# alessiodevoto/peekvit

Measured on AMD Instinct MI355X. Metric: images/sec ViT-B/16 fwd @ batch 2048, 224x224, higher is better.
Workload: dtype f16; 1 GPU; vit_b_16 forward, batch 2048/GPU, 224x224; global_batch=2048, parallelism=replicas x1 (batch-sharded, no collective), precision_mode=auto, streams=1, operands=IEEE fp16 operands, fp32 accumulate (same MFMA rate as bf16), range-guarded, range_guard_fallbacks=0

## Files before the change

peekvit_amd/csrc/pv_gemm.hip:

```cpp
#include "pv_rows.h"
#include "../../include/peekvit_hip_moe.h"
#include "pv_gelu_table.h"
#include <type_traits>
#include <cstdlib>

typedef __attribute__((ext_vector_type(8))) short s16x8;

#ifndef PV_STORE_NT
#define PV_STORE_NT 3
#endif
#define PV_STORE16(ptr, val) do { if (PV_STORE_NT & 1) __builtin_nontemporal_store((val), (ptr)); else *(ptr) = (val); } while (0)
#define PV_STORE32(ptr, val) do { if (PV_STORE_NT & 2) __builtin_nontemporal_store((val), (ptr)); else *(ptr) = (val); } while (0)
#ifndef PV_PF_MODE
#define PV_PF_MODE 2
#endif
#ifndef PV_EPI_PIPE
#define PV_EPI_PIPE 1
#endif

__device__ __forceinline__ float pv_fma_s(float a, float b, float c) {
    float r;
    asm("v_fma_f32 %0, %1, %2, %3" : "=v"(r) : "v"(a), "v"(b), "v"(c));
    return r;
}
// ... 113 lines not shown
    int fr_big;
    int gm;
    int gc;
    uint32_t* range_flag;
    float* rowsq_out;
    int res_scaled;
    int k_last;
    float* colsum_partial;
    uint16_t* x16_out;
    float* rowstat_out;
    const float* fold_stat;
    const float* fold_c1;
    const float* fold_c2;
    int ksplit;
    int k_slice;
    int64_t split_stride;
    const float* ln_gamma;
    const float* ln_beta;
    const float* ln_row_scale;
    uint16_t* ln_out;
    float ln_eps;
    const int* row_map;
    int map_rows;
#ifdef PV_STAMPS
    unsigned long long* dbg;
#endif
};

#ifdef PV_STAMPS
static unsigned long long* g_pv_dbg = nullptr;
extern "C" void pv_debug_set_stamp_buffer(void* p) { g_pv_dbg = (unsigned long long*)p; }
#define PV_STAMP(i)                                                                                  \
    do {                                                                                             \
        __builtin_amdgcn_sched_barrier(0);                                                           \
        unsigned long long t_;                                                                       \
        asm volatile("s_memtime %0\n\ts_waitcnt lgkmcnt(0)" : "=s"(t_)::"memory");                    \
        __builtin_amdgcn_sched_barrier(0);                                                           \
        if (threadIdx.x == 0 && p.dbg) p.dbg[pv_stamp_slot * 16 + (i)] = t_;                         \
    } while (0)
#else
#define PV_STAMP(i)
#endif

template <int AUX = 0>
__device__ __forceinline__ void pv_glds16(const void* gsrc, void* lds_wave_base) {
    __builtin_amdgcn_global_load_lds((const __attribute__((address_space(1))) void*)gsrc,
// ... 338 lines not shown
    static PvPerDevice attr_set;
    const int lds = 2 * 2 * G1_TILE_BYTES;
    if (attr_set.first_use()) (void)hipFuncSetAttribute(reinterpret_cast<const void*>(pv_patch_embed_kernel), hipFuncAttributeMaxDynamicSharedMemorySize, lds);
    PV_LAUNCH(pv_patch_embed_kernel, dim3((unsigned)(p.tiles_m * p.tiles_n)), dim3(256), lds, (hipStream_t)stream, p, gm);
    return pv_check_launch();
}

template <int EPI>
static int pv_launch_gemm128(const GemmDev& p, hipStream_t stream) {
    static PvPerDevice attr_set;
    const int lds = 2 * 2 * G1_TILE_BYTES;
    if (attr_set.first_use()) {
        (void)hipFuncSetAttribute(reinterpret_cast<const void*>(pv_gemm128_kernel<EPI>), hipFuncAttributeMaxDynamicSharedMemorySize, lds);
    }
    PV_LAUNCH(pv_gemm128_kernel<EPI>, dim3((unsigned)(p.tiles_m * p.tiles_n * (p.ksplit > 1 ? p.ksplit : 1))), dim3(256), lds, stream, p);
    return pv_check_launch();
}

constexpr int G2_BM = 256, G2_BN = 256, G2_BK = 64;
constexpr int G2_HALF = 128 * G2_BK * 2;
constexpr int G2_BUF = 4 * G2_HALF;
constexpr int G2_LDS = 2 * G2_BUF;

template <int EPI, bool PF = false, bool FULL = false, bool PERM = false>
__device__ __forceinline__ void pv_gemm256_tile(const GemmDev& p, char* smem, const int m0, const int n0, const bool first = true,
                                                const bool has_next = false, const int nm0 = 0, const int nn0 = 0, const int wid_pf = 0, const int slot_pf = 0) {
    int tid_ = threadIdx.x;
    if (PF) {
        int l_;
        asm volatile("v_mbcnt_lo_u32_b32 %0, -1, 0\n\tv_mbcnt_hi_u32_b32 %0, -1, %0" : "=v"(l_));
        tid_ = wid_pf * 64 + l_;
    }
    int tid = tid_, lane = tid & 63;
    const int wid = PF ? wid_pf : __builtin_amdgcn_readfirstlane(tid >> 6);
    const int wr = wid >> 2, wc = wid & 3;
#ifdef PV_STAMPS
    const size_t pv_stamp_slot = PF ? (size_t)slot_pf : (size_t)blockIdx.x;
#endif
    constexpr int PFM = PV_PF_MODE;
    constexpr int PF_BIAS_BASE = G2_LDS + ((EPI == PV_EPI_BIAS_GELU_BF16 || EPI == PV_EPI_BIAS_GELU_SPLIT_BF16 || EPI == PV_EPI_BIAS_GELU_PAIR_BF16) ? PV_GELU_CUB_N * PV_GELU_CUB_REP * 16 : 0) + 4096;
    PV_STAMP(14);
#ifdef PV_STAMPS
    if (threadIdx.x == 0 && p.dbg) { unsigned long long rt_; asm volatile("s_memrealtime %0\n\ts_waitcnt lgkmcnt(0)" : "=s"(rt_)::"memory"); p.dbg[pv_stamp_slot * 16 + 13] = rt_; }
#endif

    const int srow = wid * 8 + (lane >> 3);
    const int schunk = (lane & 7) ^ ((lane >> 3) & 7);
    const char* const a_blk = reinterpret_cast<const char*>(p.A + (int64_t)m0 * p.lda);
    const char* const w_blk = reinterpret_cast<const char*>(p.W + (int64_t)n0 * p.ldw);
// ... 12 lines not shown
    char* const lds_piece = smem + wid * 1024;
    auto stage_a = [&](int buf, int h, int kt) {
        const char* src = a_blk + kt * (G2_BK * 2);
        pv_glds16<PV_GEMM_A_AUX>(src + oa[h][0], lds_piece + buf * G2_BUF + h * G2_HALF);
        pv_glds16<PV_GEMM_A_AUX>(src + oa[h][1], lds_piece + buf * G2_BUF + h * G2_HALF + 8192);
    };
    auto stage_b = [&](int buf, int h, int kt) {
        const char* src = w_blk + kt * (G2_BK * 2);
        pv_glds16<PV_GEMM_W_AUX>(src + ow[h][0], lds_piece + buf * G2_BUF + (2 + h) * G2_HALF);
        pv_glds16<PV_GEMM_W_AUX>(src + ow[h][1], lds_piece + buf * G2_BUF + (2 + h) * G2_HALF + 8192);
    };
    auto stage_next_piece = [&](int tm0, int tn0, int pc) __attribute__((always_inline)) {
        if (pc == 8) {
            if (p.bias && wid < 4) {
                const int c_ = tn0 + wid * 64 + lane < p.N ? tn0 + wid * 64 + lane : p.N - 1;
                __builtin_amdgcn_global_load_lds((const __attribute__((address_space(1))) void*)(p.bias + c_),
                                                 (__attribute__((address_space(3))) void*)(smem + PF_BIAS_BASE + wid * 256), 4, 0, 0);
            }
            return;
        }
        const int h = (pc >> 1) & 1, jj = pc & 1;
        const int sr = wid * 8 + (lane >> 3), sc = (lane & 7) ^ ((lane >> 3) & 7);
        if (pc < 4) {
            const char* const na = reinterpret_cast<const char*>(p.A + (int64_t)tm0 * p.lda);
            int ra = h * 128 + jj * 64 + sr; ra = tm0 + ra < p.M ? ra : p.M - 1 - tm0;
            pv_glds16<PV_GEMM_A_AUX>(na + (uint32_t)(ra * (int)p.lda + sc * 8) * 2u, lds_piece + h * G2_HALF + jj * 8192);
        } else {
            const char* const nw = reinterpret_cast<const char*>(p.W + (int64_t)tn0 * p.ldw);
            const int q = jj * 64 + sr;
            int rw = h * 128 + (q & ~31) + (((q & 15) >> 2) << 3) + (((q >> 4) & 1) << 2) + (q & 3);
            rw = tn0 + rw < p.N ? rw : p.N - 1 - tn0;
            pv_glds16<PV_GEMM_W_AUX>(nw + (uint32_t)(rw * (int)p.ldw + sc * 8) * 2u, lds_piece + (2 + h) * G2_HALF + jj * 8192);
        }
    };

    typedef __attribute__((address_space(3))) const char lds_cc;
    const int frow = (lane & 15) * 128;
    const int fx0 = ((lane >> 4) ^ (lane & 7)) << 4;
    lds_cc* const lds0 = (lds_cc*)smem;
    lds_cc* a_rd[2][2];
    lds_cc* b_rd[2][2];
#pragma unroll
    for (int b = 0; b < 2; ++b)
#pragma unroll
        for (int ks = 0; ks < 2; ++ks) {
            a_rd[b][ks] = lds0 + b * G2_BUF + wr * G2_HALF + frow + (fx0 ^ (ks << 6));
            b_rd[b][ks] = lds0 + b * G2_BUF + (2 + (wc >> 1)) * G2_HALF + (wc & 1) * 8192 + frow + (fx0 ^ (ks << 6));
            asm volatile("" : "+v"(a_rd[b][ks]));
            asm volatile("" : "+v"(b_rd[b][ks]));
        }

    int en0 = n0 + wc * 64 + ((lane >> 4) << 3);
    f32x4 acc[4][8];
    if (!PF) {
#pragma unroll
        for (int i = 0; i < 4; ++i) {
            f32x4 b4 = {0.f, 0.f, 0.f, 0.f};
            if (p.bias && en0 + (i >> 1) * 32 + (i & 1) * 4 < p.N) b4 = *reinterpret_cast<const f32x4*>(p.bias + en0 + (i >> 1) * 32 + (i & 1) * 4);
#pragma unroll
            for (int j = 0; j < 8; ++j) acc[i][j] = b4;
        }
    }
    bf16x8 af[2][4][2];
    bf16x8 bfr[2][2];

#define G2_READ_A(BUF, MH)                                                                                  \
    _Pragma("unroll") for (int t_ = 0; t_ < 4; ++t_) _Pragma("unroll") for (int ks_ = 0; ks_ < 2; ++ks_)  \
        af[MH][t_][ks_] = *reinterpret_cast<const __attribute__((address_space(3))) bf16x8*>(a_rd[BUF][ks_] + ((MH) * 4 + t_) * 2048);
#define G2_READ_B(BUF, NH)                                                                                  \
    _Pragma("unroll") for (int t_ = 0; t_ < 2; ++t_) _Pragma("unroll") for (int ks_ = 0; ks_ < 2; ++ks_)  \
        bfr[t_][ks_] = *reinterpret_cast<const __attribute__((address_space(3))) bf16x8*>(b_rd[BUF][ks_] + ((NH) * 2 + t_) * 2048);
#define G2_SYNC_LOADS()                                  \
    asm volatile("s_waitcnt lgkmcnt(0)" ::: "memory");   \
    __builtin_amdgcn_s_barrier();                        \
    __builtin_amdgcn_sched_barrier(0);
#define G2_MFMA(MH, NH)                                                                                              \
    __builtin_amdgcn_s_setprio(1);                                                                                   \
    _Pragma("unroll") for (int ks_ = 0; ks_ < 2; ++ks_) _Pragma("unroll") for (int n_ = 0; n_ < 2; ++n_)            \
        _Pragma("unroll") for (int m_ = 0; m_ < 4; ++m_)                                                            \
            acc[(NH) * 2 + n_][(MH) * 4 + m_] = PV_MFMA_16x16x32(                            \
                bfr[n_][ks_], af[MH][m_][ks_], acc[(NH) * 2 + n_][(MH) * 4 + m_], 0, 0, 0);                     \
    __builtin_amdgcn_s_setprio(0);                                                                                   \
    __builtin_amdgcn_sched_barrier(0);                                                                               \
    __builtin_amdgcn_s_barrier();                                                                                    \
    __builtin_amdgcn_sched_barrier(0);

    auto ktile = [&](auto buf_c, auto sb_c, auto sa_c, int kt) {
        constexpr int BUF = decltype(buf_c)::value;
        constexpr bool SB = decltype(sb_c)::value, SA = decltype(sa_c)::value;
        G2_READ_B(BUF, 0)
        __builtin_amdgcn_sched_barrier(0);
        G2_READ_A(BUF, 0)
        if (SB) stage_b(BUF ^ 1, 0, kt + 1);
        G2_SYNC_LOADS()
        G2_MFMA(0, 0)
        G2_READ_A(BUF, 1)
        if (SB) stage_b(BUF ^ 1, 1, kt + 1);
        G2_SYNC_LOADS()
        G2_MFMA(1, 0)
        G2_READ_B(BUF, 1)
        if (SA) stage_a(BUF, 0, kt + 2);
        G2_SYNC_LOADS()
        G2_MFMA(1, 1)
        if (SA) {
            stage_a(BUF, 1, kt + 2);
            asm volatile("s_waitcnt vmcnt(4)" ::: "memory");
        } else {
            asm volatile("s_waitcnt vmcnt(0)" ::: "memory");
        }
        G2_SYNC_LOADS()
        G2_MFMA(0, 1)
    };
    using B0 = std::integral_constant<int, 0>;
    using B1 = std::integral_constant<int, 1>;
    using T = std::true_type;
    using F = std::false_type;

    const int nk = p.K / G2_BK;
    if (PF) __builtin_assume(nk >= 4);
    PV_STAMP(0);
#ifdef PV_STAMPS
    if (threadIdx.x == 0 && p.dbg) { unsigned long long rt_; asm volatile("s_memrealtime %0\n\ts_waitcnt lgkmcnt(0)" : "=s"(rt_)::"memory"); p.dbg[pv_stamp_slot * 16 + 6] = rt_; }
#endif
    const bool own_tile0 = !PF || !PFM || first;
    if (PF && (first || !PFM) && p.bias && wid < 4) {
        const int c_ = n0 + wid * 64 + lane < p.N ? n0 + wid * 64 + lane : p.N - 1;
        __builtin_amdgcn_global_load_lds((const __attribute__((address_space(1))) void*)(p.bias + c_),
                                         (__attribute__((address_space(3))) void*)(smem + PF_BIAS_BASE + wid * 256), 4, 0, 0);
    }
    if (own_tile0) { stage_a(0, 0, 0); stage_a(0, 1, 0); stage_b(0, 0, 0); stage_b(0, 1, 0); }
    stage_a(1, 0, 1); stage_a(1, 1, 1);
    constexpr bool HAS_TAB = EPI == PV_EPI_BIAS_GELU_BF16 || EPI == PV_EPI_BIAS_GELU_SPLIT_BF16 || EPI == PV_EPI_BIAS_GELU_PAIR_BF16;
    constexpr int NTAB = HAS_TAB ? 2 : 0;
    if (HAS_TAB && own_tile0) {
#pragma unroll
        for (int i = 0; i < NTAB; ++i)
            pv_glds16(reinterpret_cast<const char*>(pv_gelu_cub) + (i * 512 + tid) * 16,
                      smem + G2_LDS + (i * 512 + wid * 64) * 16);
    }
    const bool fold_dma = PV_EPI_PIPE && (EPI == PV_EPI_BIAS_BF16 || EPI == PV_EPI_BIAS_GELU_BF16) && p.fold_stat != nullptr;
    if (fold_dma) {
        constexpr int FOLD_BASE = G2_LDS + (EPI == PV_EPI_BIAS_GELU_BF16 ? PV_GELU_CUB_N * PV_GELU_CUB_REP * 16 : 0);
        const int r_ = m0 + (tid >> 1) < p.M ? m0 + (tid >> 1) : p.M - 1;
        __builtin_amdgcn_global_load_lds((const __attribute__((address_space(1))) void*)(p.fold_stat + 2 * (int64_t)r_ + (tid & 1)),
                                         (__attribute__((address_space(3))) void*)(smem + FOLD_BASE + wid * 256), 4, 0, 0);
        const int c_ = n0 + (tid & 255) < p.N ? n0 + (tid & 255) : p.N - 1;
        __builtin_amdgcn_global_load_lds((const __attribute__((address_space(1))) void*)((tid < 256 ? p.fold_c1 : p.fold_c2) + c_),
                                         (__attribute__((address_space(3))) void*)(smem + FOLD_BASE + 2048 + wid * 256), 4, 0, 0);
    }
    if (own_tile0) {
        const int inflight = 4 + NTAB + (fold_dma ? 2 : 0);
        if (inflight == 4) asm volatile("s_waitcnt vmcnt(4)" ::: "memory");
        else if (inflight == 6) asm volatile("s_waitcnt vmcnt(6)" ::: "memory");
        else if (inflight == 8) asm volatile("s_waitcnt vmcnt(8)" ::: "memory");
        else asm volatile("s_waitcnt vmcnt(10)" ::: "memory");
        __builtin_amdgcn_s_barrier();
    }
    __builtin_amdgcn_sched_barrier(0);
    PV_STAMP(1);
    if (PF) {
#pragma unroll
        for (int i = 0; i < 4; ++i) {
            f32x4 b4 = {0.f, 0.f, 0.f, 0.f};
            if (p.bias) b4 = *reinterpret_cast<const __attribute__((address_space(3))) f32x4*>((const __attribute__((address_space(3))) char*)smem + PF_BIAS_BASE + (wc * 64 + ((lane >> 4) << 3) + (i >> 1) * 32 + (i & 1) * 4) * 4);
#pragma unroll
            for (int j = 0; j < 8; ++j) acc[i][j] = b4;
        }
    }
    if (wr == 1) __builtin_amdgcn_s_barrier();

    int kt = 0;
    for (; kt + 4 <= nk; kt += 2) {
        ktile(B0{}, T{}, T{}, kt);
        ktile(B1{}, T{}, T{}, kt + 1);
    }
    ktile(B0{}, T{}, F{}, kt);
    ktile(B1{}, F{}, F{}, kt + 1);
    if (wr == 0) __builtin_amdgcn_s_barrier();
    PV_STAMP(2);
#undef G2_READ_A
#undef G2_READ_B
#undef G2_SYNC_LOADS
#undef G2_MFMA

    typedef __attribute__((address_space(3))) char lds_c;
    lds_c* const cimg = (lds_c*)smem;
    if (PF) {
        asm volatile("v_mbcnt_lo_u32_b32 %0, -1, 0\n\tv_mbcnt_hi_u32_b32 %0, -1, %0" : "=v"(lane));
        tid = wid * 64 + lane;
        en0 = n0 + wc * 64 + ((lane >> 4) << 3);
    }
    const int g = lane >> 4, i16 = lane & 15;
    const bool pf_next = PF && PFM && has_next;
    if (PFM == 1 && pf_next) {
#pragma unroll
        for (int pc = 0; pc < 9; ++pc) stage_next_piece(nm0, nn0, pc);
    }
    if (PV_EPI_PIPE && (EPI == PV_EPI_BIAS_BF16 || EPI == PV_EPI_BIAS_GELU_BF16 || EPI == PV_EPI_BIAS_GELU_PAIR_BF16)) {
        float vmax = 0.f;
        const bool fold = p.fold_stat != nullptr;
        constexpr int FOLD_BASE = G2_LDS + (EPI != PV_EPI_BIAS_BF16 ? PV_GELU_CUB_N * PV_GELU_CUB_REP * 16 : 0);
        constexpr bool PAIR2 = EPI == PV_EPI_BIAS_GELU_PAIR_BF16;
        constexpr int NU = PAIR2 ? 32 : 16;
        if (fold) {
            f32x4 k1[2][2], k2[2][2];
#pragma unroll
            for (int u = 0; u < 2; ++u)
#pragma unroll
                for (int hh = 0; hh < 2; ++hh) {
                    const int col = wc * 64 + u * 32 + g * 8 + hh * 4;
                    k1[u][hh] = *reinterpret_cast<const __attribute__((address_space(3))) f32x4*>(cimg + FOLD_BASE + 2048 + col * 4);
                    k2[u][hh] = *reinterpret_cast<const __attribute__((address_space(3))) f32x4*>(cimg + FOLD_BASE + 3072 + col * 4);
                }
#pragma unroll
            for (int mt = 0; mt < 8; ++mt) {
                const pv_f32x2_t st = *reinterpret_cast<const __attribute__((address_space(3))) pv_f32x2_t*>(cimg + FOLD_BASE + (wr * 128 + mt * 16 + i16) * 8);
                const float f_mean = st[0], f_rstd = st[1];
#pragma unroll
                for (int u = 0; u < 2; ++u)
#pragma unroll
                    for (int e = 0; e < 4; ++e) {
                        acc[2 * u][mt][e] = fmaf(f_rstd, fmaf(-f_mean, k1[u][0][e], acc[2 * u][mt][e]), k2[u][0][e]);
                        acc[2 * u + 1][mt][e] = fmaf(f_rstd, fmaf(-f_mean, k1[u][1][e], acc[2 * u + 1][mt][e]), k2[u][1][e]);
                    }
            }
        }
        PV_STAMP(8);
        const uint32_t tabc = (uint32_t)(uintptr_t)((const __attribute__((address_space(3))) f32x4*)(cimg + G2_LDS) + i16) - 0x40000000u;
        const bool ocol_ok = n0 + (lane & 31) * 8 < p.N;
        const int rb_row0 = (EPI == PV_EPI_BIAS_GELU_PAIR_BF16 ? ((wid >> 1) & 1) * 128 + (wid & 1) * 8 : (wid >> 2) * 128 + (wid & 3) * 8) + (lane >> 5);
        lds_c* const img = cimg + G2_BUF;
        const int rb_lrow0 = (wid >> 2) * 32 + (wid & 3) * 8 + (lane >> 5);
        uint32_t rb_addr[4];
#pragma unroll
        for (int j = 0; j < 4; ++j) {
            const int row = rb_lrow0 + 2 * j;
            rb_addr[j] = (uint32_t)(uintptr_t)img + row * 512 + (((lane & 31) ^ (row & 7)) << 4);
        }
        f32x4 cf[2][8];
        u32x4 rb[4];
        auto acc_unit = [&](int vn) -> int { return PAIR2 ? vn >> 1 : vn; };
        auto cf_slot = [&](int vn) -> int { return acc_unit(vn) & 1; };
        auto unit_x = [&](int vn, int e) -> float { const int n = acc_unit(vn); return acc[2 * (n & 1) + (e >> 2)][n >> 1][e & 3]; };
        auto is_gelu = [&](int vn) -> bool { return EPI == PV_EPI_BIAS_GELU_BF16 || PAIR2; };
        auto gathers = [&](int vn) -> bool { return EPI == PV_EPI_BIAS_GELU_BF16 || (PAIR2 && (vn & 1) == 0); };
        auto is_deriv = [&](int vn) -> bool { return PAIR2 && (vn & 1) == 1; };
        auto issue = [&](int vn) __attribute__((always_inline)) {
            if (gathers(vn)) {
#pragma unroll
                for (int e = 0; e < 8; e += 2) {
                    uint32_t b0, b1;
                    pv_gelu_bits2(unit_x(vn, e), unit_x(vn, e + 1), b0, b1);
                    asm volatile("ds_read_b128 %0, %1" : "=v"(cf[cf_slot(vn)][e]) : "v"((b0 << 8) + tabc));
// ... 81 lines not shown
                wait_unit(vn, PAIR2 ? vn + 2 < NU : (vn + 1 < NU && gathers(vn + 1)), vq > 0 && (vn & 3) == 0);
                finish(vn);
                if (PFM == 1 && vn == 4 && pf_next) asm volatile("s_waitcnt vmcnt(0)" ::: "memory");
                if (vq > 0) store_row(vq - 1, vn & 3);
                if ((vn & 3) == 3) {
                    asm volatile("s_waitcnt lgkmcnt(0)" ::: "memory");
                    if (vq < 4) { PV_STAMP(9 + vq); }
                    __builtin_amdgcn_s_barrier();
                    __builtin_amdgcn_sched_barrier(0);
#pragma unroll
                    for (int j = 0; j < 4; ++j)
                        asm volatile("ds_read_b128 %0, %1 offset:%2" : "=v"(rb[j]) : "v"(rb_addr[j]), "n"((vq & 1) * 32768));
                }
            }
            asm volatile("s_waitcnt lgkmcnt(0)" : "+v"(rb[0]), "+v"(rb[1]), "+v"(rb[2]), "+v"(rb[3]));
#pragma unroll
            for (int j = 0; j < 4; ++j) store_row(NU / 4 - 1, j);
        }
        pv_range_commit(vmax, p.range_flag);
    } else
    if (EPI == PV_EPI_BIAS_BF16 || EPI == PV_EPI_BIAS_GELU_BF16 || EPI == PV_EPI_BIAS_GELU_SPLIT_BF16 || EPI == PV_EPI_BIAS_GELU_PAIR_BF16) {
        constexpr bool SPLIT = EPI == PV_EPI_BIAS_GELU_SPLIT_BF16;
        constexpr bool PAIR = EPI == PV_EPI_BIAS_GELU_PAIR_BF16;
        float vmax = 0.f;
        f32x4 fc1[2][2], fc2[2][2];
        if ((EPI == PV_EPI_BIAS_BF16 || EPI == PV_EPI_BIAS_GELU_BF16) && p.fold_stat) {
#pragma unroll
            for (int u = 0; u < 2; ++u) {
                int cb = en0 + u * 32; cb = cb + 8 <= p.N ? cb : p.N - 8;
                fc1[u][0] = *reinterpret_cast<const f32x4*>(p.fold_c1 + cb); fc1[u][1] = *reinterpret_cast<const f32x4*>(p.fold_c1 + cb + 4);
                fc2[u][0] = *reinterpret_cast<const f32x4*>(p.fold_c2 + cb); fc2[u][1] = *reinterpret_cast<const f32x4*>(p.fold_c2 + cb + 4);
            }
        }
        float f_mean8[8], f_rstd8[8];
        if ((EPI == PV_EPI_BIAS_BF16 || EPI == PV_EPI_BIAS_GELU_BF16) && p.fold_stat) {
#pragma unroll
            for (int mt = 0; mt < 8; ++mt) {
                const int row_ = wr * 128 + mt * 16 + i16;
                const int mrow = m0 + row_ < p.M ? m0 + row_ : p.M - 1;
                const float2 st = *reinterpret_cast<const float2*>(p.fold_stat + 2 * (int64_t)mrow);
                f_mean8[mt] = st.x; f_rstd8[mt] = st.y;
            }
#pragma unroll
            for (int mt = 0; mt < 8; ++mt) { asm volatile("" : "+v"(f_mean8[mt])); asm volatile("" : "+v"(f_rstd8[mt])); }
        }
#pragma unroll
// ... 61 lines not shown
            asm volatile("s_waitcnt lgkmcnt(0)" ::: "memory");
            __builtin_amdgcn_s_barrier();
            uint16_t* const ob = reinterpret_cast<uint16_t*>(p.out) + n0 + (lane & 31) * 8;
#pragma unroll
            for (int j = 0; j < 16; ++j) {
                const int row = wid * 32 + 2 * j + (lane >> 5);
                const u32x4 v = *reinterpret_cast<const __attribute__((address_space(3))) u32x4*>(cimg + row * 512 + (((lane & 31) ^ (row & 7)) << 4));
                if (m0 + row < p.M && n0 + (lane & 31) * 8 < p.N) {
                    uint16_t* o = ob + (int64_t)(m0 + row) * p.ldo;
                    if (PAIR) {
                        *reinterpret_cast<u32x4*>(pass == 0 ? o + p.N : o) = v;
                    } else if (!SPLIT) {
                        *reinterpret_cast<u32x4*>(o) = v;
                    } else if (pass == 0) {
                        *reinterpret_cast<u32x4*>(o) = v;
                        *reinterpret_cast<u32x4*>(o + 2 * p.N) = v;
                    } else {
                        *reinterpret_cast<u32x4*>(o + p.N) = v;
                    }
                }
            }
        }
        if (!SPLIT) pv_range_commit(vmax, p.range_flag);
    } else {
        constexpr bool DG = EPI == PV_EPI_GELU_GRAD_BF16;
        float cs8[DG ? 8 : 1];
        if constexpr (DG) {
#pragma unroll
            for (int e = 0; e < 8; ++e) cs8[e] = 0.f;
        }
        u32x4 dg[DG ? 2 : 1][DG ? 4 : 1];
        const int dg_col = n0 + 8 * (lane & 31);
        const bool dg_col_ok = FULL || dg_col + 8 <= p.N;
        float vmax = 0.f;
        lds_c* const img = cimg + G2_BUF;
        const bool col_ok = FULL || n0 + lane * 4 < p.N;
        const int ncol = col_ok ? n0 + lane * 4 : 0;
        f32x4 rr[2][8];
        float rsc[2] = {1.0f, 1.0f};
        auto row_of = [&](int q, int j) -> int64_t {
            int m = m0 + q * 64 + wid * 8 + j;
            m = (FULL || m < p.M) ? m : p.M - 1;
            if (PERM) return p.row_map[m];
            if (EPI == PV_EPI_BIAS_POS_F32) { const int img_ = m / p.rpi, pi = m - img_ * p.rpi; return (int64_t)img_ * p.rpo + p.row_off + pi; }
            return m;
        };
// ... 8 lines not shown
                return;
            }
#pragma unroll
            for (int j = 0; j < 8; ++j) {
                int m = m0 + q * 64 + wid * 8 + j;
                m = (FULL || m < p.M) ? m : p.M - 1;
                f32x4& r = rr[q & 1][j];
                if (EPI == PV_EPI_BIAS_F32) {
                    r = (f32x4){0.f, 0.f, 0.f, 0.f};
                } else if (EPI == PV_EPI_BIAS_RES_F32) {
                    int64_t rm = m;
                    if (PERM) { const int s_ = p.row_map[m]; rm = (s_ >= 0 && s_ < p.map_rows) ? s_ : 0; }
                    r = *reinterpret_cast<const f32x4*>(p.res + rm * p.ldr + ncol);
                } else {
                    const int img_ = m / p.rpi, pi = m - img_ * p.rpi;
                    r = *reinterpret_cast<const f32x4*>(p.pos + (int64_t)(p.row_off + pi) * p.N + ncol);
                }
            }
            if (EPI == PV_EPI_BIAS_RES_F32 && p.row_scale) {
                int m = m0 + q * 64 + wid * 8 + (lane & 7);
                rsc[q & 1] = p.row_scale[m < p.M ? m : p.M - 1];
            }
        };
        fetch(0);
        fetch(1);
        if (PFM == 2 && pf_next) {
#pragma unroll
            for (int pc = 0; pc < 9; ++pc) stage_next_piece(nm0, nn0, pc);
        }
#pragma unroll
        for (int q = 0; q < 4; ++q) {
            if (q > 0) __builtin_amdgcn_s_barrier();
            if (wr == (q >> 1)) {
#pragma unroll
                for (int ml = 0; ml < 4; ++ml) {
                    const int mt = 4 * (q & 1) + ml, row = ml * 16 + i16;
#pragma unroll
                    for (int nt = 0; nt < 4; ++nt) {
                        const int c = wc * 16 + (nt >> 1) * 8 + g * 2 + (nt & 1);
                        *reinterpret_cast<__attribute__((address_space(3))) f32x4*>(img + row * 1024 + ((c ^ (i16 & 7)) << 4)) = acc[nt][mt];
                    }
                }
            }
            asm volatile("s_waitcnt lgkmcnt(0)" ::: "memory");
            __builtin_amdgcn_s_barrier();
            if (PFM == 1 && q == 0 && pf_next) asm volatile("s_waitcnt vmcnt(0)" ::: "memory");
            float fs[8], fq[8];
            if constexpr (DG) {
#pragma unroll
                for (int jj = 0; jj < 4; ++jj) {
                    const int row = wid * 8 + 2 * jj + (lane >> 5), c0 = 2 * (lane & 31);
                    const f32x4 va = *reinterpret_cast<const __attribute__((address_space(3))) f32x4*>(img + row * 1024 + ((c0 ^ (row & 7)) << 4));
                    const f32x4 vb = *reinterpret_cast<const __attribute__((address_space(3))) f32x4*>(img + row * 1024 + (((c0 + 1) ^ (row & 7)) << 4));
                    const u32x4 d = dg[q & 1][jj];
                    const u32x4 pk = {pv_pack_bf16x2(pv_mul_s(va[0], pv_unpack_lo(d[0])), pv_mul_s(va[1], pv_unpack_hi(d[0]))),
                                      pv_pack_bf16x2(pv_mul_s(va[2], pv_unpack_lo(d[1])), pv_mul_s(va[3], pv_unpack_hi(d[1]))),
                                      pv_pack_bf16x2(pv_mul_s(vb[0], pv_unpack_lo(d[2])), pv_mul_s(vb[1], pv_unpack_hi(d[2]))),
                                      pv_pack_bf16x2(pv_mul_s(vb[2], pv_unpack_lo(d[3])), pv_mul_s(vb[3], pv_unpack_hi(d[3])))};
                    const int mrow = m0 + q * 64 + row;
// ... 15 lines not shown
                const f32x4 r = rr[q & 1][j];
                const float sc = (EPI == PV_EPI_BIAS_RES_F32 && p.row_scale)
                                     ? __builtin_bit_cast(float, __builtin_amdgcn_readlane(__builtin_bit_cast(int, rsc[q & 1]), j)) : 1.0f;
                f32x4 o;
                if (EPI == PV_EPI_BIAS_F32) {
                    const float qs = ncol < p.qcols ? p.qscale : 1.0f;
                    o = (f32x4){v[0] * qs, v[1] * qs, v[2] * qs, v[3] * qs};
                } else if (EPI == PV_EPI_BIAS_RES_F32) {
                    const float tr = p.res_scaled ? sc : 1.0f;
                    o = (f32x4){fmaf(sc, v[0], tr * r[0]), fmaf(sc, v[1], tr * r[1]), fmaf(sc, v[2], tr * r[2]), fmaf(sc, v[3], tr * r[3])};
                }
                else o = (f32x4){r[0] + v[0], r[1] + v[1], r[2] + v[2], r[3] + v[3]};
                const bool ok = (FULL || (m0 + q * 64 + row < p.M && col_ok)) && (!PERM || (orow >= 0 && orow < p.map_rows));
                if (ok) PV_STORE32(reinterpret_cast<f32x4*>(reinterpret_cast<float*>(p.out) + orow * p.ldo + ncol), o);
                if (EPI == PV_EPI_BIAS_RES_F32 && p.rowsq_out)
                    fq[j] = ok ? pv_add_s(pv_add_s(o[0] * o[0], o[1] * o[1]), pv_add_s(o[2] * o[2], o[3] * o[3])) : 0.f;
                if (EPI == PV_EPI_BIAS_RES_F32 && p.x16_out) {
                    if (ok)
                        PV_STORE16(reinterpret_cast<u32x2*>(p.x16_out + orow * (int64_t)p.N + ncol), ((u32x2){pv_pack_bf16x2_tracked(o[0], o[1], vmax), pv_pack_bf16x2_tracked(o[2], o[3], vmax)}));
                    fs[j] = ok ? pv_add_s(pv_add_s(o[0], o[1]), pv_add_s(o[2], o[3])) : 0.f;
                    fq[j] = ok ? pv_add_s(pv_add_s(o[0] * o[0], o[1] * o[1]), pv_add_s(o[2] * o[2], o[3] * o[3])) : 0.f;
                }
            }
            if (q + 2 < 4) fetch(q + 2);
            {
                const int r_ = (lane >> 3) & 7, mrow = m0 + q * 64 + wid * 8 + r_;
                if (EPI == PV_EPI_BIAS_RES_F32 && p.rowsq_out && !p.x16_out) {
                    const float tq = pv_reduce8_rows(fq, lane);
                    if ((lane & 7) == 0 && mrow < p.M) p.rowsq_out[(int64_t)(n0 / G2_BN) * p.M + mrow] = tq;
                }
                if (EPI == PV_EPI_BIAS_RES_F32 && p.x16_out) {
                    const float ts = pv_reduce8_rows(fs, lane), tq = pv_reduce8_rows(fq, lane);
                    if ((lane & 7) == 0 && mrow < p.M)
                        *reinterpret_cast<float2*>(p.rowstat_out + ((int64_t)(n0 / G2_BN) * p.M + mrow) * 2) = make_float2(ts, tq);
                }
            }
        }
        if (EPI == PV_EPI_BIAS_RES_F32 && p.x16_out) pv_range_commit(vmax, p.range_flag);
        if (EPI == PV_EPI_GELU_GRAD_BF16 && p.colsum_partial) {
            asm volatile("s_waitcnt lgkmcnt(0)" ::: "memory");
            __builtin_amdgcn_s_barrier();
            if constexpr (DG) {
#pragma unroll
                for (int e = 0; e < 8; ++e) cs8[e] = pv_add_s(cs8[e], __shfl_xor(cs8[e], 32, 64));
                if (lane < 32) {
                    *reinterpret_cast<__attribute__((address_space(3))) f32x4*>(cimg + G2_BUF + wid * 1024 + lane * 32) = (f32x4){cs8[0], cs8[1], cs8[2], cs8[3]};
                    *reinterpret_cast<__attribute__((address_space(3))) f32x4*>(cimg + G2_BUF + wid * 1024 + lane * 32 + 16) = (f32x4){cs8[4], cs8[5], cs8[6], cs8[7]};
                }
            }
            asm volatile("s_waitcnt lgkmcnt(0)" ::: "memory");
            __builtin_amdgcn_s_barrier();
            if (tid < 256 && n0 + tid < p.N) {
                float t = 0.f;
#pragma unroll
                for (int w = 0; w < 8; ++w) t += *reinterpret_cast<const __attribute__((address_space(3))) float*>(cimg + G2_BUF + w * 1024 + tid * 4);
                p.colsum_partial[(int64_t)(m0 / G2_BM) * p.N + n0 + tid] = t;
            }
        }
    }
    if (PFM == 2 && pf_next) {
        const bool full = FULL || (m0 + G2_BM <= p.M && n0 + G2_BN <= p.N);
        constexpr bool B16 = EPI == PV_EPI_BIAS_BF16 || EPI == PV_EPI_BIAS_GELU_BF16 || EPI == PV_EPI_BIAS_GELU_PAIR_BF16 || EPI == PV_EPI_GELU_GRAD_BF16;
        if (!full) asm volatile("s_waitcnt vmcnt(0)" ::: "memory");
        else if (B16) asm volatile("s_waitcnt vmcnt(16)" ::: "memory");
        else asm volatile("s_waitcnt vmcnt(32)" ::: "memory");
    }
    PV_STAMP(3);
#ifdef PV_STAMPS
    if (threadIdx.x == 0 && p.dbg) {
        unsigned hw, xcc;
        asm volatile("s_getreg_b32 %0, hwreg(HW_REG_HW_ID)" : "=s"(hw));
        asm volatile("s_getreg_b32 %0, hwreg(HW_REG_XCC_ID)" : "=s"(xcc));
        p.dbg[pv_stamp_slot * 16 + 5] = ((unsigned long long)(xcc & 0xf) << 32) | hw;
    }
    asm volatile("s_waitcnt vmcnt(0)" ::: "memory");
    PV_STAMP(4);
    if (threadIdx.x == 0 && p.dbg) { unsigned long long rt_; asm volatile("s_memrealtime %0\n\ts_waitcnt lgkmcnt(0)" : "=s"(rt_)::"memory"); p.dbg[pv_stamp_slot * 16 + 7] = rt_; }
#endif
}

template <int EPI>
__global__ __launch_bounds__(512) void pv_gemm256_kernel(const GemmDev p_in) {
    extern __shared__ __attribute__((aligned(16))) char smem[];
    GemmDev p = p_in;
// ... 17 lines not shown
    else pv_gemm256_tile<EPI, false, false>(p, smem, m0, n0);
}

template <int EPI>
__global__ __launch_bounds__(512) void pv_gemm256_pf_kernel(const GemmDev p) {
    extern __shared__ __attribute__((aligned(16))) char smem[];
    const int ntiles = p.tiles_m * p.tiles_n;
    const int xcd = blockIdx.x & 7, j = blockIdx.x >> 3, per = gridDim.x >> 3;
    const int q8 = ntiles >> 3, r8 = ntiles & 7;
    const int start = xcd < r8 ? xcd * (q8 + 1) : r8 * (q8 + 1) + (xcd - r8) * q8;
    const int cnt = q8 + (xcd < r8 ? 1 : 0);
    const int nfull = p.tiles_n / p.gc;
    auto decode = [&](int tile, int& m0, int& n0) {
        const int ch = min(tile / (p.gc * p.tiles_m), nfull);
        const int r = tile - ch * p.gc * p.tiles_m;
        const int cw = ch < nfull ? p.gc : p.tiles_n - nfull * p.gc;
        const int grp = r / (p.gm * cw), rem = r - grp * (p.gm * cw);
        const int gsz = min(p.gm, p.tiles_m - grp * p.gm);
        const int tnl = rem / gsz, tm = grp * p.gm + (rem - tnl * gsz);
        m0 = tm * G2_BM; n0 = (ch * p.gc + tnl) * G2_BN;
    };
    const int wid = __builtin_amdgcn_readfirstlane((int)threadIdx.x >> 6);
    int m0 = 0, n0 = 0, nm0 = 0, nn0 = 0;
    if (j < cnt) decode(start + j, m0, n0);
    for (int i = j; i < cnt; i += per) {
        const bool has_next = i + per < cnt;
        if (has_next) decode(start + i + per, nm0, nn0);
        if (m0 + G2_BM <= p.M && n0 + G2_BN <= p.N) pv_gemm256_tile<EPI, true, true>(p, smem, m0, n0, i == j, has_next, nm0, nn0, wid, start + i);
        else pv_gemm256_tile<EPI, true, false>(p, smem, m0, n0, i == j, has_next, nm0, nn0, wid, start + i);
        asm volatile("s_waitcnt lgkmcnt(0)" ::: "memory");
        __builtin_amdgcn_s_barrier();
        __builtin_amdgcn_sched_barrier(0);
        m0 = nm0; n0 = nn0;
    }
}

struct PvGroupDev {
    const int* tile_expert;
    int64_t w_stride;
    int E;
};

template <int EPI>
__global__ __launch_bounds__(512) void pv_gemm256_kernel(const GemmDev p_in, const PvGroupDev g) {
    extern __shared__ __attribute__((aligned(16))) char smem[];
    const int ntiles = p_in.tiles_m * p_in.tiles_n;
    const int tile = pv_xcd_remap(blockIdx.x, ntiles);
    const int tm = tile / p_in.tiles_n, tn = tile - tm * p_in.tiles_n;
    const int e = __builtin_amdgcn_readfirstlane(g.tile_expert[tm]);
    if (e < 0 || e >= g.E) return;
    GemmDev p = p_in;
    p.W += (int64_t)e * g.w_stride;
    if (p.bias) p.bias += (int64_t)e * p.N;
    const int m0 = tm * G2_BM, n0 = tn * G2_BN;
    constexpr bool PERM = EPI == PV_EPI_BIAS_RES_F32;
    if (n0 + G2_BN <= p.N) pv_gemm256_tile<EPI, false, true, PERM>(p, smem, m0, n0);
// ... 263 lines not shown
        asm volatile("s_waitcnt lgkmcnt(0)" ::: "memory");
        __builtin_amdgcn_s_barrier();
    }
    asm volatile("s_waitcnt vmcnt(0)" ::: "memory");
    __builtin_amdgcn_s_barrier();
    const int nch = (p.N / 4 + 63) / 64;
    if (nch <= 1) pv_fused_ln_rows<1>(p, m0);
    else if (nch == 2) pv_fused_ln_rows<2>(p, m0);
    else if (nch == 3) pv_fused_ln_rows<3>(p, m0);
    else if (nch == 4) pv_fused_ln_rows<4>(p, m0);
    else if (nch <= 8) pv_fused_ln_rows<8>(p, m0);
    else pv_fused_ln_rows<16>(p, m0);
}

#ifndef PV_GEMM_PF_DEFAULT
#define PV_GEMM_PF_DEFAULT 1
#endif
static int g_pv_pf = -1;
extern "C" void pv_debug_set_gemm_pf(int on) { g_pv_pf = on; }
static bool pv_gemm_pf_enabled() {
    static const int env = [] { const char* e = getenv("PV_GEMM_PF"); return e ? atoi(e) : PV_GEMM_PF_DEFAULT; }();
    return g_pv_pf >= 0 ? g_pv_pf != 0 : env != 0;
}
static int pv_cu_count() {
    static int cached[64] = {};
    int d = 0;
    if (hipGetDevice(&d) != hipSuccess || d < 0 || d >= 64) return 0;
    if (cached[d] == 0) {
        int n = 0;
        if (hipDeviceGetAttribute(&n, hipDeviceAttributeMultiprocessorCount, d) != hipSuccess) n = 0;
        cached[d] = n > 0 ? n : -1;
    }
    return cached[d] > 0 ? cached[d] : 0;
}

template <int EPI>
static int pv_launch_gemm256(const GemmDev& p, hipStream_t stream) {
    static PvPerDevice attr_set;
    constexpr int lds = G2_LDS + ((EPI == PV_EPI_BIAS_GELU_BF16 || EPI == PV_EPI_BIAS_GELU_SPLIT_BF16 || EPI == PV_EPI_BIAS_GELU_PAIR_BF16)
                                        ? PV_GELU_CUB_N * PV_GELU_CUB_REP * 16 : 0)
                        + ((EPI == PV_EPI_BIAS_BF16 || EPI == PV_EPI_BIAS_GELU_BF16) ? 4096 : 0);
    constexpr int lds_pf = EPI == PV_EPI_GELU_GRAD_BF16 ? lds
                         : G2_LDS + ((EPI == PV_EPI_BIAS_GELU_BF16 || EPI == PV_EPI_BIAS_GELU_SPLIT_BF16 || EPI == PV_EPI_BIAS_GELU_PAIR_BF16) ? PV_GELU_CUB_N * PV_GELU_CUB_REP * 16 : 0) + 4096 + 1024;
    constexpr bool PF_OK = EPI != PV_EPI_BIAS_GELU_SPLIT_BF16 && (PV_EPI_PIPE || (EPI != PV_EPI_BIAS_BF16 && EPI != PV_EPI_BIAS_GELU_BF16 && EPI != PV_EPI_BIAS_GELU_PAIR_BF16));
    if (attr_set.first_use()) {
        (void)hipFuncSetAttribute(reinterpret_cast<const void*>(static_cast<void (*)(const GemmDev)>(pv_gemm256_kernel<EPI>)), hipFuncAttributeMaxDynamicSharedMemorySize, lds);
        if (PF_OK) (void)hipFuncSetAttribute(reinterpret_cast<const void*>(pv_gemm256_pf_kernel<EPI>), hipFuncAttributeMaxDynamicSharedMemorySize, lds_pf);
    }
    if (PF_OK) {
        const int cus = pv_cu_count();
        if (pv_gemm_pf_enabled() && p.ksplit <= 1 && p.K >= 4 * G2_BK && (int64_t)p.tiles_m * p.tiles_n >= 2 * (int64_t)cus && cus >= 8 &&
            !(EPI == PV_EPI_GELU_GRAD_BF16 && p.bias)) {
            PV_LAUNCH(pv_gemm256_pf_kernel<EPI>, dim3((unsigned)(cus & ~7)), dim3(512), lds_pf, stream, p);
            return pv_check_launch();
        }
    }
    PV_LAUNCH((static_cast<void (*)(const GemmDev)>(pv_gemm256_kernel<EPI>)), dim3((unsigned)(p.tiles_m * p.tiles_n * (p.ksplit > 1 ? p.ksplit : 1))), dim3(512), lds, stream, p);
    return pv_check_launch();
}

template <int EPI>
static int pv_launch_gemm256_rows(const GemmDev& p, hipStream_t stream) {
    static PvPerDevice attr_set;
    if (attr_set.first_use()) {
        (void)hipFuncSetAttribute(reinterpret_cast<const void*>(pv_gemm256_rows_kernel<EPI>), hipFuncAttributeMaxDynamicSharedMemorySize, G2_LDS);
    }
    PV_LAUNCH(pv_gemm256_rows_kernel<EPI>, dim3((unsigned)p.tiles_m), dim3(512), G2_LDS, stream, p);
    return pv_check_launch();
}

template <int N_>
__device__ __forceinline__ void pv_wait_vmcnt() { asm volatile("s_waitcnt vmcnt(%0)" ::"n"(N_) : "memory"); }

struct PvFrCounts { int pro; int v[3][4]; };
constexpr PvFrCounts pv_fr_counts(int NPH, int PW, int AP = 2) {
    constexpr int NK = 8;
// ... 598 lines not shown
```

Measured before the change: 27970 images/sec.

## Split persistent GEMM tail wave into half-height tiles across idle workgroups

Result: no change. 27990 images/sec, median of 2 (+0.1%).

```diff
diff --git a/peekvit_amd/csrc/pv_gemm.hip b/peekvit_amd/csrc/pv_gemm.hip
--- a/peekvit_amd/csrc/pv_gemm.hip
+++ b/peekvit_amd/csrc/pv_gemm.hip
@@ -159,6 +159,7 @@
     float ln_eps;
     const int* row_map;
     int map_rows;
+    int half_tail;
 #ifdef PV_STAMPS
     unsigned long long* dbg;
 #endif
@@ -543,9 +544,17 @@
 constexpr int G2_BUF = 4 * G2_HALF;
 constexpr int G2_LDS = 2 * G2_BUF;
 
-template <int EPI, bool PF = false, bool FULL = false, bool PERM = false>
+constexpr bool pv_gemm256_half_ok(int epi) {
+    return epi == PV_EPI_BIAS_RES_F32 || epi == PV_EPI_BIAS_POS_F32 || epi == PV_EPI_BIAS_F32 ||
+           (PV_EPI_PIPE && (epi == PV_EPI_BIAS_BF16 || epi == PV_EPI_BIAS_GELU_BF16));
+}
+
+template <int EPI, bool PF = false, bool FULL = false, bool PERM = false, bool HALF = false>
 __device__ __forceinline__ void pv_gemm256_tile(const GemmDev& p, char* smem, const int m0, const int n0, const bool first = true,
-                                                const bool has_next = false, const int nm0 = 0, const int nn0 = 0, const int wid_pf = 0, const int slot_pf = 0) {
+                                                const int has_next = 0, const int nm0 = 0, const int nn0 = 0, const int wid_pf = 0, const int slot_pf = 0) {
+    static_assert(!HALF || (PF && !PERM && pv_gemm256_half_ok(EPI)), "half tiles: the persistent launch's tail only");
+    constexpr int MT = HALF ? 4 : 8;
+    constexpr int RW = HALF ? 64 : 128;
     int tid_ = threadIdx.x;
     if (PF) {
         int l_;
@@ -604,6 +613,7 @@
         const int h = (pc >> 1) & 1, jj = pc & 1;
         const int sr = wid * 8 + (lane >> 3), sc = (lane & 7) ^ ((lane >> 3) & 7);
         if (pc < 4) {
+            if (h == 1 && has_next == 2) return;
             const char* const na = reinterpret_cast<const char*>(p.A + (int64_t)tm0 * p.lda);
             int ra = h * 128 + jj * 64 + sr; ra = tm0 + ra < p.M ? ra : p.M - 1 - tm0;
             pv_glds16<PV_GEMM_A_AUX>(na + (uint32_t)(ra * (int)p.lda + sc * 8) * 2u, lds_piece + h * G2_HALF + jj * 8192);
@@ -626,24 +636,24 @@
     for (int b = 0; b < 2; ++b)
 #pragma unroll
         for (int ks = 0; ks < 2; ++ks) {
-            a_rd[b][ks] = lds0 + b * G2_BUF + wr * G2_HALF + frow + (fx0 ^ (ks << 6));
+            a_rd[b][ks] = lds0 + b * G2_BUF + wr * (HALF ? G2_HALF / 2 : G2_HALF) + frow + (fx0 ^ (ks << 6));
             b_rd[b][ks] = lds0 + b * G2_BUF + (2 + (wc >> 1)) * G2_HALF + (wc & 1) * 8192 + frow + (fx0 ^ (ks << 6));
             asm volatile("" : "+v"(a_rd[b][ks]));
             asm volatile("" : "+v"(b_rd[b][ks]));
         }
 
     int en0 = n0 + wc * 64 + ((lane >> 4) << 3);
-    f32x4 acc[4][8];
+    f32x4 acc[4][MT];
     if (!PF) {
 #pragma unroll
         for (int i = 0; i < 4; ++i) {
             f32x4 b4 = {0.f, 0.f, 0.f, 0.f};
             if (p.bias && en0 + (i >> 1) * 32 + (i & 1) * 4 < p.N) b4 = *reinterpret_cast<const f32x4*>(p.bias + en0 + (i >> 1) * 32 + (i & 1) * 4);
 #pragma unroll
-            for (int j = 0; j < 8; ++j) acc[i][j] = b4;
-        }
-    }
-    bf16x8 af[2][4][2];
+            for (int j = 0; j < MT; ++j) acc[i][j] = b4;
+        }
+    }
+    bf16x8 af[HALF ? 1 : 2][4][2];
     bf16x8 bfr[2][2];
 
 #define G2_READ_A(BUF, MH)                                                                                  \
@@ -670,6 +680,23 @@
     auto ktile = [&](auto buf_c, auto sb_c, auto sa_c, int kt) {
         constexpr int BUF = decltype(buf_c)::value;
         constexpr bool SB = decltype(sb_c)::value, SA = decltype(sa_c)::value;
+        if constexpr (HALF) {
+            G2_READ_B(BUF, 0)
+            __builtin_amdgcn_sched_barrier(0);
+            G2_READ_A(BUF, 0)
+            if (SB) { stage_b(BUF ^ 1, 0, kt + 1); stage_b(BUF ^ 1, 1, kt + 1); }
+            G2_SYNC_LOADS()
+            G2_MFMA(0, 0)
+            G2_READ_B(BUF, 1)
+            if (SA) {
+                stage_a(BUF, 0, kt + 2);
+                asm volatile("s_waitcnt vmcnt(2)" ::: "memory");
+            } else {
+                asm volatile("s_waitcnt vmcnt(0)" ::: "memory");
+            }
+            G2_SYNC_LOADS()
+            G2_MFMA(0, 1)
+        } else {
         G2_READ_B(BUF, 0)
         __builtin_amdgcn_sched_barrier(0);
         G2_READ_A(BUF, 0)
@@ -692,6 +719,7 @@
         }
         G2_SYNC_LOADS()
         G2_MFMA(0, 1)
+        }
     };
     using B0 = std::integral_constant<int, 0>;
     using B1 = std::integral_constant<int, 1>;
@@ -710,8 +738,8 @@
         __builtin_amdgcn_global_load_lds((const __attribute__((address_space(1))) void*)(p.bias + c_),
                                          (__attribute__((address_space(3))) void*)(smem + PF_BIAS_BASE + wid * 256), 4, 0, 0);
     }
-    if (own_tile0) { stage_a(0, 0, 0); stage_a(0, 1, 0); stage_b(0, 0, 0); stage_b(0, 1, 0); }
-    stage_a(1, 0, 1); stage_a(1, 1, 1);
+    if (own_tile0) { stage_a(0, 0, 0); if (!HALF) stage_a(0, 1, 0); stage_b(0, 0, 0); stage_b(0, 1, 0); }
+    stage_a(1, 0, 1); if (!HALF) stage_a(1, 1, 1);
     constexpr bool HAS_TAB = EPI == PV_EPI_BIAS_GELU_BF16 || EPI == PV_EPI_BIAS_GELU_SPLIT_BF16 || EPI == PV_EPI_BIAS_GELU_PAIR_BF16;
     constexpr int NTAB = HAS_TAB ? 2 : 0;
     if (HAS_TAB && own_tile0) {
@@ -731,8 +759,9 @@
                                          (__attribute__((address_space(3))) void*)(smem + FOLD_BASE + 2048 + wid * 256), 4, 0, 0);
     }
     if (own_tile0) {
-        const int inflight = 4 + NTAB + (fold_dma ? 2 : 0);
-        if (inflight == 4) asm volatile("s_waitcnt vmcnt(4)" ::: "memory");
+        const int inflight = (HALF ? 2 : 4) + NTAB + (fold_dma ? 2 : 0);
+        if (inflight == 2) asm volatile("s_waitcnt vmcnt(2)" ::: "memory");
+        else if (inflight == 4) asm volatile("s_waitcnt vmcnt(4)" ::: "memory");
         else if (inflight == 6) asm volatile("s_waitcnt vmcnt(6)" ::: "memory");
         else if (inflight == 8) asm volatile("s_waitcnt vmcnt(8)" ::: "memory");
         else asm volatile("s_waitcnt vmcnt(10)" ::: "memory");
@@ -746,7 +775,7 @@
             f32x4 b4 = {0.f, 0.f, 0.f, 0.f};
             if (p.bias) b4 = *reinterpret_cast<const __attribute__((address_space(3))) f32x4*>((const __attribute__((address_space(3))) char*)smem + PF_BIAS_BASE + (wc * 64 + ((lane >> 4) << 3) + (i >> 1) * 32 + (i & 1) * 4) * 4);
 #pragma unroll
-            for (int j = 0; j < 8; ++j) acc[i][j] = b4;
+            for (int j = 0; j < MT; ++j) acc[i][j] = b4;
         }
     }
     if (wr == 1) __builtin_amdgcn_s_barrier();
@@ -773,7 +802,7 @@
         en0 = n0 + wc * 64 + ((lane >> 4) << 3);
     }
     const int g = lane >> 4, i16 = lane & 15;
-    const bool pf_next = PF && PFM && has_next;
+    const bool pf_next = PF && PFM && has_next != 0;
     if (PFM == 1 && pf_next) {
 #pragma unroll
         for (int pc = 0; pc < 9; ++pc) stage_next_piece(nm0, nn0, pc);
@@ -783,7 +812,7 @@
         const bool fold = p.fold_stat != nullptr;
         constexpr int FOLD_BASE = G2_LDS + (EPI != PV_EPI_BIAS_BF16 ? PV_GELU_CUB_N * PV_GELU_CUB_REP * 16 : 0);
         constexpr bool PAIR2 = EPI == PV_EPI_BIAS_GELU_PAIR_BF16;
-        constexpr int NU = PAIR2 ? 32 : 16;
+        constexpr int NU = PAIR2 ? 32 : 2 * MT;
         if (fold) {
             f32x4 k1[2][2], k2[2][2];
 #pragma unroll
@@ -795,8 +824,8 @@
                     k2[u][hh] = *reinterpret_cast<const __attribute__((address_space(3))) f32x4*>(cimg + FOLD_BASE + 3072 + col * 4);
                 }
 #pragma unroll
-            for (int mt = 0; mt < 8; ++mt) {
-                const pv_f32x2_t st = *reinterpret_cast<const __attribute__((address_space(3))) pv_f32x2_t*>(cimg + FOLD_BASE + (wr * 128 + mt * 16 + i16) * 8);
+            for (int mt = 0; mt < MT; ++mt) {
+                const pv_f32x2_t st = *reinterpret_cast<const __attribute__((address_space(3))) pv_f32x2_t*>(cimg + FOLD_BASE + (wr * RW + mt * 16 + i16) * 8);
                 const float f_mean = st[0], f_rstd = st[1];
 #pragma unroll
                 for (int u = 0; u < 2; ++u)
@@ -810,7 +839,7 @@
         PV_STAMP(8);
         const uint32_t tabc = (uint32_t)(uintptr_t)((const __attribute__((address_space(3))) f32x4*)(cimg + G2_LDS) + i16) - 0x40000000u;
         const bool ocol_ok = n0 + (lane & 31) * 8 < p.N;
-        const int rb_row0 = (EPI == PV_EPI_BIAS_GELU_PAIR_BF16 ? ((wid >> 1) & 1) * 128 + (wid & 1) * 8 : (wid >> 2) * 128 + (wid & 3) * 8) + (lane >> 5);
+        const int rb_row0 = (EPI == PV_EPI_BIAS_GELU_PAIR_BF16 ? ((wid >> 1) & 1) * 128 + (wid & 1) * 8 : (wid >> 2) * RW + (wid & 3) * 8) + (lane >> 5);
         lds_c* const img = cimg + G2_BUF;
         const int rb_lrow0 = (wid >> 2) * 32 + (wid & 3) * 8 + (lane >> 5);
         uint32_t rb_addr[4];
@@ -938,6 +967,7 @@
     if (EPI == PV_EPI_BIAS_BF16 || EPI == PV_EPI_BIAS_GELU_BF16 || EPI == PV_EPI_BIAS_GELU_SPLIT_BF16 || EPI == PV_EPI_BIAS_GELU_PAIR_BF16) {
         constexpr bool SPLIT = EPI == PV_EPI_BIAS_GELU_SPLIT_BF16;
         constexpr bool PAIR = EPI == PV_EPI_BIAS_GELU_PAIR_BF16;
+        if constexpr (!HALF) {
         float vmax = 0.f;
         f32x4 fc1[2][2], fc2[2][2];
         if ((EPI == PV_EPI_BIAS_BF16 || EPI == PV_EPI_BIAS_GELU_BF16) && p.fold_stat) {
@@ -1045,6 +1075,7 @@
             }
         }
         if (!SPLIT) pv_range_commit(vmax, p.range_flag);
+        }
     } else {
         constexpr bool DG = EPI == PV_EPI_GELU_GRAD_BF16;
         float cs8[DG ? 8 : 1];
@@ -1099,6 +1130,7 @@
                 rsc[q & 1] = p.row_scale[m < p.M ? m : p.M - 1];
             }
         };
+        constexpr int NPASS = HALF ? 2 : 4;
         fetch(0);
         fetch(1);
         if (PFM == 2 && pf_next) {
@@ -1106,12 +1138,12 @@
             for (int pc = 0; pc < 9; ++pc) stage_next_piece(nm0, nn0, pc);
         }
 #pragma unroll
-        for (int q = 0; q < 4; ++q) {
+        for (int q = 0; q < NPASS; ++q) {
             if (q > 0) __builtin_amdgcn_s_barrier();
-            if (wr == (q >> 1)) {
+            if (wr == (HALF ? q : q >> 1)) {
 #pragma unroll
                 for (int ml = 0; ml < 4; ++ml) {
-                    const int mt = 4 * (q & 1) + ml, row = ml * 16 + i16;
+                    const int mt = HALF ? ml : 4 * (q & 1) + ml, row = ml * 16 + i16;
 #pragma unroll
                     for (int nt = 0; nt < 4; ++nt) {
                         const int c = wc * 16 + (nt >> 1) * 8 + g * 2 + (nt & 1);
@@ -1173,7 +1205,7 @@
                     fq[j] = ok ? pv_add_s(pv_add_s(o[0] * o[0], o[1] * o[1]), pv_add_s(o[2] * o[2], o[3] * o[3])) : 0.f;
                 }
             }
-            if (q + 2 < 4) fetch(q + 2);
+            if (q + 2 < NPASS) fetch(q + 2);
             {
                 const int r_ = (lane >> 3) & 7, mrow = m0 + q * 64 + wid * 8 + r_;
                 if (EPI == PV_EPI_BIAS_RES_F32 && p.rowsq_out && !p.x16_out) {
@@ -1210,7 +1242,7 @@
         }
     }
     if (PFM == 2 && pf_next) {
-        const bool full = FULL || (m0 + G2_BM <= p.M && n0 + G2_BN <= p.N);
+        const bool full = !HALF && (FULL || (m0 + G2_BM <= p.M && n0 + G2_BN <= p.N));
         constexpr bool B16 = EPI == PV_EPI_BIAS_BF16 || EPI == PV_EPI_BIAS_GELU_BF16 || EPI == PV_EPI_BIAS_GELU_PAIR_BF16 || EPI == PV_EPI_GELU_GRAD_BF16;
         if (!full) asm volatile("s_waitcnt vmcnt(0)" ::: "memory");
         else if (B16) asm volatile("s_waitcnt vmcnt(16)" ::: "memory");
@@ -1274,16 +1306,34 @@
     };
     const int wid = __builtin_amdgcn_readfirstlane((int)threadIdx.x >> 6);
     int m0 = 0, n0 = 0, nm0 = 0, nn0 = 0;
-    if (j < cnt) decode(start + j, m0, n0);
-    for (int i = j; i < cnt; i += per) {
-        const bool has_next = i + per < cnt;
+    constexpr bool HALF_OK = pv_gemm256_half_ok(EPI);
+    const int L = cnt % per;
+    const bool split = HALF_OK && p.half_tail && L > 0 && 2 * L <= per;
+    const int cnt_full = split ? cnt - L : cnt;
+    const int hidx = (split && j < 2 * L) ? start + cnt_full + (j >> 1) : -1;
+    if (j < cnt_full) decode(start + j, m0, n0);
+    else if (hidx >= 0) { decode(hidx, m0, n0); m0 += (j & 1) * (G2_BM / 2); }
+    for (int i = j; i < cnt_full; i += per) {
+        int has_next = i + per < cnt_full ? 1 : 0;
         if (has_next) decode(start + i + per, nm0, nn0);
+        else if (hidx >= 0) {
+            decode(hidx, nm0, nn0);
+            nm0 += (j & 1) * (G2_BM / 2);
+            if (nm0 < p.M) has_next = 2;
+        }
         if (m0 + G2_BM <= p.M && n0 + G2_BN <= p.N) pv_gemm256_tile<EPI, true, true>(p, smem, m0, n0, i == j, has_next, nm0, nn0, wid, start + i);
         else pv_gemm256_tile<EPI, true, false>(p, smem, m0, n0, i == j, has_next, nm0, nn0, wid, start + i);
         asm volatile("s_waitcnt lgkmcnt(0)" ::: "memory");
         __builtin_amdgcn_s_barrier();
         __builtin_amdgcn_sched_barrier(0);
         m0 = nm0; n0 = nn0;
+    }
+    if constexpr (HALF_OK) {
+        if (hidx >= 0 && m0 < p.M) {
+            const int hslot = ntiles + (hidx << 1) + (j & 1);
+            if (m0 + G2_BM / 2 <= p.M && n0 + G2_BN <= p.N) pv_gemm256_tile<EPI, true, true, false, true>(p, smem, m0, n0, j >= cnt_full, 0, 0, 0, wid, hslot);
+            else pv_gemm256_tile<EPI, true, false, false, true>(p, smem, m0, n0, j >= cnt_full, 0, 0, 0, wid, hslot);
+        }
     }
 }
 
@@ -1593,6 +1643,10 @@
     static const int env = [] { const char* e = getenv("PV_GEMM_PF"); return e ? atoi(e) : PV_GEMM_PF_DEFAULT; }();
     return g_pv_pf >= 0 ? g_pv_pf != 0 : env != 0;
 }
+static bool pv_gemm_half_tail_enabled() {
+    static const int env = [] { const char* e = getenv("PV_GEMM_HALF_TAIL"); return e ? atoi(e) : 1; }();
+    return env != 0;
+}
 static int pv_cu_count() {
     static int cached[64] = {};
     int d = 0;
@@ -1622,7 +1676,9 @@
         const int cus = pv_cu_count();
         if (pv_gemm_pf_enabled() && p.ksplit <= 1 && p.K >= 4 * G2_BK && (int64_t)p.tiles_m * p.tiles_n >= 2 * (int64_t)cus && cus >= 8 &&
             !(EPI == PV_EPI_GELU_GRAD_BF16 && p.bias)) {
-            PV_LAUNCH(pv_gemm256_pf_kernel<EPI>, dim3((unsigned)(cus & ~7)), dim3(512), lds_pf, stream, p);
+            GemmDev pp = p;
+            pp.half_tail = pv_gemm_half_tail_enabled() ? 1 : 0;
+            PV_LAUNCH(pv_gemm256_pf_kernel<EPI>, dim3((unsigned)(cus & ~7)), dim3(512), lds_pf, stream, pp);
             return pv_check_launch();
         }
     }
```
